# alberto-paparella/MusicRecommendation

Hardware: AMD Instinct MI355X
Metric: scored (test-user,song) pairs/sec, ItemBasedModel, 1/2/4/8 MI355X + mAP@10 (higher is better)
Workload: dtype int64

## Files before the change

include/mr_engine.h:

```cpp
#ifndef MR_ENGINE_H
#define MR_ENGINE_H

#include <stdint.h>
#include <stddef.h>

#ifdef __cplusplus
extern "C" {
#endif

#define MR_OK          0
#define MR_E_INVALID  -1
#define MR_E_HIP      -2
#define MR_E_OOM      -3
#define MR_E_STATE    -4
#define MR_E_IO       -5
#define MR_E_PARSE    -6
#define MR_E_RCCL     -7

#define MR_UBM 0
#define MR_IBM 1

#define MR_OUT_F32 0
#define MR_OUT_F64 1

// ... 17 lines not shown
  int32_t song_lo;
  int32_t song_hi;
  int32_t block_songs;
  int32_t out_dtype;
  int32_t topk;
  int32_t dense;
  int32_t time_kernels;
  int32_t stage1;
  int32_t stage1_chunk;
  int32_t train_order;
  int32_t topk_lists;
  int32_t ibm_route;
  int32_t reserved[2];
} mr_options;

typedef struct mr_ctx mr_ctx;

int mr_options_default(mr_options* opt);

int mr_create(const mr_options* opt, mr_ctx** out);
int mr_destroy(mr_ctx* ctx);

int mr_load(mr_ctx* ctx, const mr_dataset* d);

int mr_shard_info(const mr_ctx* ctx, int32_t* song_lo, int32_t* song_hi, int32_t* n_test_users);

int mr_launch_info(const mr_ctx* ctx, int32_t* shape, int32_t* block_songs, int32_t* n_tiles);

int mr_batch_info(const mr_ctx* ctx, int32_t* batch, int32_t* chunk, int32_t* n_chunks);

int mr_route_info(const mr_ctx* ctx, int32_t* route, int32_t* n_rows, int64_t* pool_entries);

int mr_topk_mode(const mr_ctx* ctx, int32_t* candidate_only);

int mr_cooc_stats(mr_ctx* ctx, int64_t* index_nnz, int64_t* consumed, int64_t* build_reads);

typedef struct mr_cooc_bytes_t {
  int64_t heavy_rows, light_rows;
  int64_t heavy_reads, light_reads;
  int64_t heavy_index_bytes, light_index_bytes;
  int64_t heavy_visits;
  int64_t consumed_bytes;
  int64_t group_tiles;
  int64_t n_groups;
  int64_t index_sparse_entries, index_dense_songs;
  int64_t consumed_sparse_entries, consumed_dense_songs;
} mr_cooc_bytes_t;
int mr_cooc_bytes(mr_ctx* ctx, mr_cooc_bytes_t* out);

int mr_shard_tile_songs(const mr_options* opt, int32_t n_train_users, int32_t n_test_users,
                        int32_t* tile_songs);

int mr_shard_tile_songs_n(const mr_options* opt, int32_t n_train_users, int32_t n_test_users, int32_t n_songs,
                          int32_t n_shards, int32_t* tile_songs);

int mr_run(mr_ctx* ctx, int model);
int mr_sync(mr_ctx* ctx);

int mr_graph_capture(mr_ctx* ctx, int model, int32_t n_steps);
int mr_graph_launch(mr_ctx* ctx);

int mr_device_outputs(const mr_ctx* ctx, void** dense, int32_t** topk_songs,
                      int64_t** topk_keys, double** topk_scores);

int mr_run_into(mr_ctx* ctx, int model, void* dense_dev);

// ... 125 lines not shown
```

musicrecommendation_amd/_lib.py:

```python
from __future__ import annotations

import ctypes
import os
from ctypes import POINTER, c_char_p, c_double, c_int, c_int32, c_int64, c_void_p

_HERE = os.path.dirname(os.path.abspath(__file__))
_VARIANT = os.environ.get("MR_ENGINE_LIB", "")
LIB_PATH = os.path.join(_HERE, f"libmr_engine_{_VARIANT}.so" if _VARIANT else "libmr_engine.so")

MR_OK = 0
MR_E_INVALID = -1
MR_E_HIP = -2
MR_E_OOM = -3
MR_E_STATE = -4
MR_E_IO = -5
MR_E_PARSE = -6
MR_E_RCCL = -7
MR_TRANSPORT_AUTO, MR_TRANSPORT_COPY, MR_TRANSPORT_RCCL = 0, 1, 2
MR_UBM = 0
MR_IBM = 1
STAGE1 = {"auto": 0, "fused": 1, "separate": 2, "wide": 4}
SHAPES = {0: "separate", 1: "fused", 3: "wide"}
MR_OUT_F32 = 0
MR_OUT_F64 = 1
# ... 67 lines not shown
        ("te_songs", c_void_p),
        ("stream", c_void_p),
    ]


class MrCoocBytes(ctypes.Structure):
    _fields_ = [(n, c_int64) for n in ("heavy_rows", "light_rows", "heavy_reads", "light_reads",
                                       "heavy_index_bytes", "light_index_bytes", "heavy_visits", "consumed_bytes",
                                       "group_tiles", "n_groups", "index_sparse_entries", "index_dense_songs",
                                       "consumed_sparse_entries", "consumed_dense_songs")]


MR_COMB_LINEAR = 0
MR_COMB_AGGREGATION = 1
MR_COMB_STOCHASTIC = 2


class EngineError(RuntimeError):
    def __init__(self, code: int, where: str, msg: str):
        super().__init__(f"{where}: {_ERRNAMES.get(code, code)}: {msg}")
        self.code = code


SIGNATURES = {
    "mr_options_default": (c_int, [POINTER(MrOptions)]),
    "mr_create": (c_int, [POINTER(MrOptions), POINTER(c_void_p)]),
    "mr_destroy": (c_int, [c_void_p]),
    "mr_load": (c_int, [c_void_p, POINTER(MrDataset)]),
    "mr_shard_info": (c_int, [c_void_p, POINTER(c_int32), POINTER(c_int32), POINTER(c_int32)]),
    "mr_launch_info": (c_int, [c_void_p, POINTER(c_int32), POINTER(c_int32), POINTER(c_int32)]),
    "mr_batch_info": (c_int, [c_void_p, POINTER(c_int32), POINTER(c_int32), POINTER(c_int32)]),
    "mr_route_info": (c_int, [c_void_p, POINTER(c_int32), POINTER(c_int32), POINTER(c_int64)]),
    "mr_topk_mode": (c_int, [c_void_p, POINTER(c_int32)]),
    "mr_cooc_stats": (c_int, [c_void_p, POINTER(c_int64), POINTER(c_int64), POINTER(c_int64)]),
    "mr_cooc_bytes": (c_int, [c_void_p, POINTER(MrCoocBytes)]),
    "mr_shard_tile_songs": (c_int, [POINTER(MrOptions), c_int32, c_int32, POINTER(c_int32)]),
    "mr_shard_tile_songs_n": (c_int, [POINTER(MrOptions), c_int32, c_int32, c_int32, c_int32, POINTER(c_int32)]),
    "mr_run": (c_int, [c_void_p, c_int]),
    "mr_sync": (c_int, [c_void_p]),
    "mr_graph_capture": (c_int, [c_void_p, c_int, c_int32]),
    "mr_graph_launch": (c_int, [c_void_p]),
    "mr_device_outputs": (c_int, [c_void_p, POINTER(c_void_p), POINTER(c_void_p), POINTER(c_void_p), POINTER(c_void_p)]),
    "mr_score_dense": (c_int, [c_void_p, c_int, c_void_p]),
    "mr_topk": (c_int, [c_void_p, c_int, c_int, c_void_p, c_void_p, c_void_p]),
    "mr_copy_dense": (c_int, [c_void_p, c_void_p]),
    "mr_copy_topk": (c_int, [c_void_p, c_void_p, c_void_p, c_void_p]),
    "mr_copy_topk_device": (c_int, [c_void_p, c_void_p, c_void_p]),
    "mr_copy_topk_device_async": (c_int, [c_void_p, c_void_p, c_void_p]),
    "mr_topk_merge_device_async": (c_int, [c_void_p, c_int32, c_int32, c_int32, c_void_p, c_void_p, c_void_p, c_void_p,
                                           c_void_p]),
    "mr_topk_record_bytes": (c_int, [c_int32, c_int32, POINTER(c_int64)]),
    "mr_topk_merge_records_async": (c_int, [c_void_p, c_int32, c_int32, c_int32, c_void_p, c_int64, c_void_p, c_void_p,
                                            c_void_p]),
    "mr_topk_merge_host": (c_int, [c_int32, c_int32, c_int32, c_void_p, c_void_p, c_void_p, c_void_p, c_void_p, c_void_p]),
    "mr_topk_merge_device": (c_int, [c_void_p, c_int32, c_int32, c_int32, c_void_p, c_void_p, c_void_p, c_void_p, c_void_p, c_void_p]),
    "mr_kernel_times": (c_int, [c_void_p, c_int32, POINTER(c_int64), POINTER(c_double), c_int32]),
    "mr_debug_stamps": (c_int, [c_void_p, c_void_p, c_int64]),
    "mr_timing_begin": (c_int, [c_void_p]),
    "mr_timing_stop": (c_int, [c_void_p]),
    "mr_timing_end": (c_int, [c_void_p, POINTER(c_int64), POINTER(c_double)]),
    "mr_stream": (c_void_p, [c_void_p]),
    "mr_run_into": (c_int, [c_void_p, c_int, c_void_p]),
    "mr_view_get": (c_int, [c_void_p, POINTER(MrView)]),
    "mr_topk_dense_device": (c_int, [c_void_p, c_void_p, c_int32]),
    "mr_combine_device": (c_int, [c_void_p, c_int, c_double, ctypes.c_uint64, c_int64, c_int64, c_void_p, c_void_p, c_void_p]),
    "mr_combine_all_device": (c_int, [c_void_p, c_double, c_double, c_double, ctypes.c_uint64, c_int64, c_int64,
# ... 78 lines not shown
```

musicrecommendation_amd/csrc/mr_engine.hip:

```cpp
#include <hip/hip_runtime.h>

#include <algorithm>
#include <atomic>
#include <climits>
#include <cmath>
#include <cstdarg>
#include <cstdio>
#include <cstdlib>
#include <cstring>
#include <limits>
#include <mutex>
#include <string>
#include <vector>

#ifndef MR_TILE_ROWS
#define MR_TILE_ROWS 32
#endif

#include "mr_engine.h"
#include "mr_internal.h"
#include "mr_par.h"


namespace {
// ... 893 lines not shown
  const uint2* te_sched;
  const long long* sched_off;
  const double* sqrt_c;
  const long long* trs_off;
  const int* trs_users;
  const long long* q_song;
  const double* sqrt_tr;
  const double* sqrt_te;
  int cap;
  int chunk, n_chunks;
  int n_users, xcd_remap;
  int merge_rows;
  const int* nbr_v;
  const long long* nbr_q;
  const int* nbr_cnt;
  void* dense_out;
  long long* cand_key;
  int* cand_song;
  unsigned* counter;
  long long* top_key;
  int* top_song;
  double* top_score;
  long long* stamps;
  int topk_lists;
  int n_rows, nseg;
  const int* te_row;
  const long long* seg_off;
  const int* seg_len;
  const unsigned* pool;
  unsigned long long* mm_key;
  int mm_n;
  int cand;
  const float* rsq_c;
};

template <int MODEL, typename OutT, bool FUSED>
__global__ __launch_bounds__(kThreads) void k_score(ScoreParams p) {
  extern __shared__ __align__(16) unsigned char smem_raw[];
  const int bs = p.block_songs;
  const ScoreLds L = score_lds(bs, FUSED ? p.n_tr : 0, p.topk, p.n_tiles, FUSED ? 0 : p.n_chunks);
  unsigned long long* acc = reinterpret_cast<unsigned long long*>(smem_raw + L.acc);
  unsigned* heard = reinterpret_cast<unsigned*>(smem_raw + L.heard);
  long long* wk = reinterpret_cast<long long*>(smem_raw + L.wk);
  int* ws = reinterpret_cast<int*>(smem_raw + L.ws);
  long long* fk = reinterpret_cast<long long*>(smem_raw + L.fk);
  int* fs = reinterpret_cast<int*>(smem_raw + L.fs);
  int* flag = reinterpret_cast<int*>(smem_raw + L.flag);

  int tile = blockIdx.x;
  int bu = blockIdx.y;
  if (p.xcd_remap) {
    const int lin = blockIdx.y * gridDim.x + blockIdx.x;
    const int slot = lin >> 3;
    bu = (slot / p.n_tiles) * 8 + (lin & 7);
    tile = slot % p.n_tiles;
    if (bu >= p.n_users) return;
  }
  const int u = p.user0 + bu;
  const int tid = threadIdx.x;
  const int blo = p.song_lo + tile * bs;
  const int bhi = min(p.song_hi, blo + bs);
  const int bw = bhi - blo;
  const double two_f = ldexp(1.0, p.frac_bits);
#ifdef MR_STAMPS
  long long* sb = p.stamps ? p.stamps + ((size_t)blockIdx.y * gridDim.x + blockIdx.x) * kStampSlots : nullptr;
#endif
// ... 668 lines not shown
      ba = a > ba ? a : ba;
      ap[e] = a;
    }
  }
  const long long mk = be >= 0 ? (long long)__float_as_uint(ba) : kKeyNone;
  const int ms = be >= 0 ? blo + tid + be * NT : INT_MAX;
  MR_STAMP(3);
  long long tk;
  int tsg;
  block_tau<NT, NG>(k, mk, ms, gm, tk, tsg, sb);
  int* counter = reinterpret_cast<int*>(reinterpret_cast<long long*>(gm) + NG + 1) + NG + 1;
  int* crank = counter + 1 + NG;
  const float thr = __uint_as_float((unsigned)tk) * (1.f - 0x1p-17f);
  const double inv_f = ldexp(1.0, -p.frac_bits);
  unsigned sm = 0u;
#pragma unroll
  for (int e = 0; e < EMAX; ++e) sm |= ap[e] >= thr ? 1u << e : 0u;
  while (sm) {
    const int e = __builtin_ctz(sm);
    sm &= sm - 1u;
    const int i = tid + e * NT;
    double score = (double)(long long)acc[i] * inv_f;
    if (MODEL == MR_IBM) score = score / p.sqrt_c[blo + i];
    const int pos = atomicAdd(counter, 1);
    if (pos < cap) { ck[pos] = __double_as_longlong(score); cs[pos] = blo + i; }
  }
  __syncthreads();
  stamp_at(sb, 11);
  const int nc = *counter;
  if (nc > cap) return false;
  rank_survivors<NT>(nc, k, ck, cs, crank, fk, fs);
  return true;
}
constexpr int kCandE = 20;

template <int MODEL, typename OutT, int NT, int KS, bool COOC>
__global__ __launch_bounds__(NT) void k_score_wide(ScoreParams p) {
  constexpr int NW = NT / 64;
  extern __shared__ __align__(16) unsigned char smem_raw[];
  const int bs = p.block_songs;
  const WideLds<NT> L = wide_lds<NT>(bs, p.topk, p.n_chunks);
  unsigned long long* acc = reinterpret_cast<unsigned long long*>(smem_raw + L.acc);
  unsigned* heard = reinterpret_cast<unsigned*>(smem_raw + L.heard);
  int* cpre = reinterpret_cast<int*>(smem_raw + L.cpre);
  int* s_scan = reinterpret_cast<int*>(smem_raw + L.s_scan);

  const int lin = blockIdx.y * gridDim.x + blockIdx.x;
  const int slot = lin >> 3;
  int bu, tile;
  if (p.xcd_remap == 2) {
    const int per_xcd = (gridDim.x * gridDim.y) >> 3;
    const int pidx = (lin & 7) * per_xcd + slot;
    tile = pidx / gridDim.y;
    bu = pidx - tile * gridDim.y;
  } else if (p.xcd_remap == 3) {
    tile = lin / gridDim.y;
    bu = lin - tile * gridDim.y;
  } else {
    bu = (slot / p.n_tiles) * 8 + (lin & 7);
    tile = slot % p.n_tiles;
  }
  if (bu >= p.n_users) return;
  const int u = p.user0 + bu;
  const int tid = threadIdx.x, lane = tid & 63, w = tid >> 6;
  const int blo = p.song_lo + tile * bs;
  const int bhi = min(p.song_hi, blo + bs);
  const int bw = bhi - blo;
  MR_STAMP(0);

  constexpr bool kPF = COOC && MR_COOC_PF > 0;
  constexpr int PF = kPF ? MR_COOC_PF : 1;
  double scp[PF];
  if constexpr (kPF) {
#pragma unroll
    for (int e = 0; e < PF; ++e) {
      const int i = tid + e * NT;
      scp[e] = i < bw ? p.sqrt_c[blo + i] : 1.0;
    }
  }
  constexpr bool kDPF = COOC && MR_COOC_DPF;
  int pf_r = -1, pf_s = 0, pf_sl = 0;
  long long pf_off = 0;
  unsigned long long pf_q = 0ull;
  if constexpr (kDPF) {
    const long long a = p.te_off[u];
    if (tid < min<long long>(p.nseg, p.te_off[u + 1] - a)) {
      pf_r = p.te_row[a + tid];
      pf_s = p.te_songs[a + tid];
    }
  }
  auto zero_acc = [&]() {
#if MR_WIDE_Z16
    for (int i = tid; 2 * i < bw; i += NT) reinterpret_cast<ulonglong2*>(acc)[i] = make_ulonglong2(0ull, 0ull);
#else
    for (int i = tid; i < bw; i += NT) acc[i] = 0ull;
#endif
  };
  if (!(COOC && MR_COOC_NOZERO) || p.te_off[u + 1] == p.te_off[u]) zero_acc();
  if constexpr (kDPF) {
    if (pf_r >= 0) {
      pf_sl = p.seg_len[(size_t)tile * p.n_rows + pf_r];
      pf_off = p.seg_off[(size_t)tile * p.n_rows + pf_r];
      pf_q = (unsigned long long)p.q_song[pf_s];
    }
  }
  for (int i = tid; i < bs / 32; i += NT) heard[i] = 0u;
  __syncthreads();
  for (long long i = p.te_off[u] + tid; i < p.te_off[u + 1]; i += NT) {
    const int s = p.te_songs[i];
    if (s >= blo && s < bhi) atomicOr(&heard[(s - blo) >> 5], 1u << ((s - blo) & 31));
  }
  const int nch = p.n_chunks;
  int cnt = 0;
  if constexpr (!COOC) {
    for (int c0 = 0; c0 < nch; c0 += NT) {
      const int cc = c0 + tid;
      const int x = cc < nch ? p.nbr_cnt[(size_t)bu * nch + cc] : 0;
      int tot;
      const int pre = block_excl_scan_nt<NT>(x, &tot, s_scan);
      if (cc < nch) cpre[cc] = cnt + pre;
      cnt += tot;
    }
    if (tid == 0) cpre[nch] = cnt;
  }
  __syncthreads();
  MR_STAMP(1);

  bool have_rv = false;
  float pre_rv[MR_CAND_EB];
  if constexpr (COOC) {
    long long* m_off = reinterpret_cast<long long*>(smem_raw + L.wk);
    unsigned long long* m_q = reinterpret_cast<unsigned long long*>(m_off + p.nseg);
    long long* d_off = reinterpret_cast<long long*>(m_q + p.nseg);
    unsigned long long* d_q = reinterpret_cast<unsigned long long*>(d_off + p.nseg);
    int* m_pre = reinterpret_cast<int*>(d_q + p.nseg);
    int* d_fmt = m_pre + p.nseg + 1;
    const long long t0 = p.te_off[u], t1 = p.te_off[u + 1];
    const int* slen = p.seg_len + (size_t)tile * p.n_rows;
    const long long* soff = p.seg_off + (size_t)tile * p.n_rows;
    for (long long c0 = t0; c0 < t1; c0 += p.nseg) {
      const int ns = (int)min<long long>(p.nseg, t1 - c0);
      int len = 0, isd = 0, fmt = 0;
      long long off = 0, tail_off = -1;
      unsigned long long q = 0ull;
      if (tid < ns) {
        int r, sl = 0;
        if (kDPF && c0 == t0) {
          r = pf_r;
          sl = pf_sl;
          off = pf_off;
          q = pf_q;
        } else {
          r = p.te_row[c0 + tid];
          if (r >= 0) {
            sl = slen[r];
            off = soff[r];
            q = (unsigned long long)p.q_song[p.te_songs[c0 + tid]];
          }
        }
// ... 201 lines not shown
    int cur = 0;
    auto load_list = [&](int k0, int (&v)[R], unsigned long long (&q)[R]) {
#pragma unroll
      for (int r = 0; r < R; ++r) {
        const int k = k0 + r * NT;
        v[r] = -1;
        q[r] = 0ull;
        if (k < cnt) {
          while (cur + 1 < nch && cpre[cur + 1] <= k) ++cur;
          const size_t idx = (size_t)cur * p.chunk + (k - cpre[cur]);
          v[r] = nv[idx];
          q[r] = (unsigned long long)nq[idx];
        }
      }
    };
    walk_tile_lists<NT, R, kSeg, unsigned long long>(tid, cnt, load_list, p.toff + (size_t)tile * p.n_tr, p.tsongs,
                                                     [&](unsigned x, unsigned long long q) { atomicAdd(&acc[x], q); });
  }
  __syncthreads();
  MR_STAMP(2);

  long long* wk = reinterpret_cast<long long*>(smem_raw + L.wk);
  int* ws = reinterpret_cast<int*>(smem_raw + L.ws);
  long long* fk = reinterpret_cast<long long*>(smem_raw + L.fk);
  int* fs = reinterpret_cast<int*>(smem_raw + L.fs);
  const int k = KS == 10 ? 10 : p.topk;
  bool have = false;
#ifdef MR_STAMPS
  long long* sbp = p.stamps ? p.stamps + ((size_t)blockIdx.y * gridDim.x + blockIdx.x) * kStampSlots : nullptr;
#else
  long long* sbp = nullptr;
#endif
  if (p.cand) {
    have = wide_cand_topk<MODEL, NT, kCandE>(p, acc, heard, blo, bw, k, smem_raw + L.gm, wk, ws,
                                             min(256, NW * k), fk, fs, sbp, have_rv, pre_rv);
    MR_STAMP(6);
  }
  if (!have) {
  const double inv_f = ldexp(1.0, -p.frac_bits);
  OutT* out = reinterpret_cast<OutT*>(p.dense_out) + (size_t)u * p.width + (blo - p.song_lo);
  long long mk = kKeyNone;
  int ms = INT_MAX;
  OutT lmn = (OutT)INFINITY, lmx = (OutT)-INFINITY;
  auto store = [&](int i, bool h, double score) {
    const OutT o = h ? (OutT)NAN : (OutT)score;
    out[i] = o;
    if (!h) {
      lmn = o < lmn ? o : lmn;
      lmx = o > lmx ? o : lmx;
    }
  };
  constexpr int EB = MR_WIDE_EB;
  int i_start = tid;
  if constexpr (kPF) {
#pragma unroll
    for (int e = 0; e < PF; ++e) {
      const int i = tid + e * NT;
      if (i >= bw) continue;
      const bool h = (heard[i >> 5] >> (i & 31)) & 1u;
      double score = (double)(long long)acc[i] * inv_f;
      score = score / scp[e];
      if (p.dense) store(i, h, score);
      const long long key = h ? kKeyNone : __double_as_longlong(score);
      acc[i] = (unsigned long long)key;
      if (key >= 0) take_if_before(mk, ms, key, blo + i);
    }
    i_start = tid + PF * NT;
  }
// ... 1157 lines not shown

}

struct mr_ctx {
  mr_options opt{};
  int dev_share = 1;
  hipStream_t stream = nullptr;
  bool loaded = false;
  bool ran = false;
  bool fused = false;
  int shape = kShapeSeparate;
  int last_model = -1;
  int n_tr = 0, n_te = 0, n_s = 0;
  int song_lo = 0, song_hi = 0, width = 0;
  int block_songs = 0, n_tiles = 0;
  int cap = 0, batch = 0;
  int chunk = 1, n_chunks = 1;
  size_t score_lds = 0, nbr_lds = 0, merge_lds = 0, wide_lds = 0;
  ScoreKernel score_kernel[2] = {nullptr, nullptr};
  NbrKernel nbr_kernel[2] = {nullptr, nullptr};
  DevBuf<long long> tr_off, te_off, trs_off, q_song, cand_key, top_key, nbr_q;
  DevBuf<int> te_songs, trs_users, toff, nbr_v, nbr_cnt, cand_song, top_song;
  DevBuf<unsigned short> tsongs;
  DevBuf<unsigned> tpack;
  DevBuf<int2> te_rng;
  DevBuf<long long> te_q;
  DevBuf<uint2> te_sched;
  DevBuf<long long> sched_off;
  DevBuf<int> sbound;
  DevBuf<unsigned> counter;
  DevBuf<double> sqrt_c, sqrt_tr, sqrt_te, top_score;
  DevBuf<float> rsq_c;
  bool cand_on = false;
  DevBuf<unsigned char> dense;
  DevBuf<long long> stamps;
  hipEvent_t stage_ev[2] = {nullptr, nullptr};
  static constexpr int kRing = 1024;
  std::vector<hipEvent_t> ring;
  int ring_used = 0;
  bool ring_has_stage1[kRing] = {};
  long long launches[3] = {0, 0, 0};
  double ms[3] = {0, 0, 0};
  hipEvent_t win[2] = {nullptr, nullptr};
  bool win_open = false;
  bool win_stopped = false;
  void* dense_override = nullptr;
  DevBuf<unsigned long long> mm_key;
  bool mm_on = false, mm_valid = false;
  hipGraph_t graph = nullptr;
  hipGraphExec_t graph_exec = nullptr;
  int graph_steps = 0;
  DevBuf<unsigned> flag;
  long long win_launches = 0;
  int ibm_route = 1;
  int cooc_nt = 1024;
  size_t cooc_score_lds = 0;
  int n_rows = 0, nseg = 0;
  long long pool_cap = 0;
  size_t cooc_lds = 0;
  ScoreKernel cooc_kernel = nullptr;
  DevBuf<int> row_song, te_row, seg_len;
  DevBuf<long long> row_base, seg_off;
  DevBuf<unsigned> pool;
  DevBuf<unsigned> row_nnz;
  std::vector<int32_t> row_users;
  std::vector<int64_t> row_reads;
  std::vector<int32_t> row_listeners;
  std::vector<uint8_t> row_light;
  long long build_reads = 0;
  bool cooc_ran = false;
  hipStream_t side[2] = {nullptr, nullptr};
  hipEvent_t side_fork = nullptr, side_join[2] = {nullptr, nullptr};
  int n_heavy = 0, n_light = 0;
  int n_light_tier[6] = {0, 0, 0, 0, 0, 0};
  int n_heavy32 = 0;
  int n_big16 = 0, tcap16 = 0, tcap32 = 0;
  int dense_div = 0, force32 = 0;
  unsigned sat = 255;
  size_t bstamp_off = 0;
  size_t lstamp_off = 0;
  DevBuf<int> rows_order, row_slots;
  DevBuf<int4> rdesc;
  DevBuf<long long> sr_off;
  DevBuf<unsigned> sr_songs;
  DevBuf<unsigned> urec;
  DevBuf<unsigned> lrec;
  DevBuf<uint2> llrec;
  int grp = 0, n_grp = 0, urec_words = 0, lrec_words = 0;
  int group_nt = 1024;

  void release_data() {
    tr_off.release(); te_off.release(); trs_off.release(); q_song.release();
    cand_key.release(); top_key.release(); nbr_q.release();
    tsongs.release(); tpack.release(); te_rng.release(); te_q.release(); te_sched.release(); sched_off.release(); te_songs.release(); trs_users.release(); toff.release(); sbound.release();
    nbr_v.release(); nbr_cnt.release(); cand_song.release(); top_song.release();
    counter.release();
    sqrt_c.release(); sqrt_tr.release(); sqrt_te.release(); top_score.release();
    rsq_c.release(); cand_on = false;
    dense.release();
    mm_key.release(); mm_on = mm_valid = false;
    stamps.release();
    flag.release();
    row_song.release(); te_row.release(); seg_len.release(); row_base.release(); seg_off.release();
    pool.release();
    rows_order.release(); row_slots.release(); sr_off.release(); sr_songs.release(); row_nnz.release();
    urec.release(); lrec.release(); llrec.release(); rdesc.release(); grp = n_grp = urec_words = lrec_words = 0;
    row_users.clear(); row_reads.clear(); row_listeners.clear(); row_light.clear();
    build_reads = 0; cooc_ran = false;
    ibm_route = 1; n_rows = 0; nseg = 0; pool_cap = 0; cooc_kernel = nullptr; n_heavy = n_light = n_heavy32 = 0;
    for (int& x : n_light_tier) x = 0;
    if (graph_exec) (void)hipGraphExecDestroy(graph_exec);
    if (graph) (void)hipGraphDestroy(graph);
    graph_exec = nullptr;
    graph = nullptr;
    graph_steps = 0;
    loaded = ran = false;
  }
};

namespace {

template <class F>
int64_t first_bad(int64_t n, F&& bad, int64_t grain = 1 << 14) {
  std::atomic<int64_t> best{INT64_MAX};
  mr_par::parallel_for(n, [&](int64_t lo, int64_t hi, int) {
    for (int64_t i = lo; i < hi && i < best.load(std::memory_order_relaxed); ++i)
      if (bad(i)) {
        int64_t cur = best.load();
        while (i < cur && !best.compare_exchange_weak(cur, i)) {}
        return;
      }
// ... 824 lines not shown
        c->urec.release();
      }
      MR_HIP(hipStreamSynchronize(st));
    }
  }
  if (k > 0) {
    const int cand_users = !wide ? n_te : route == 2 ? std::max(batch, std::min(n_te, 65528)) : batch;
    const size_t nc = (size_t)cand_users * n_tiles * k;
    if ((rc = dev_alloc(c->cand_key, nc))) return rc;
    if ((rc = dev_alloc(c->cand_song, nc))) return rc;
    const size_t nk = (size_t)n_te * k;
    if ((rc = dev_alloc(c->top_key, (size_t)topk_record_bytes(nk) / 8))) return rc;
    c->top_song.p = reinterpret_cast<int*>(c->top_key.p + nk);
    c->top_song.n = nk;
    c->top_song.own = false;
    if ((rc = dev_alloc(c->top_score, (size_t)n_te * k))) return rc;
    const size_t n_ctr = wide ? (size_t)n_te : (size_t)n_te * kCounterStride;
    if ((rc = dev_alloc(c->counter, n_ctr))) return rc;
    MR_HIP(hipMemsetAsync(c->counter.p, 0, n_ctr * sizeof(unsigned), st));
  }
  const size_t esz = c->opt.out_dtype == MR_OUT_F64 ? 8 : 4;
  if ((rc = dev_alloc(c->dense, c->opt.dense ? (size_t)n_te * width * esz : 1))) return rc;
  if ((rc = dev_alloc(c->flag, 1))) return rc;

  c->fused = fused;
  c->shape = shape;
  c->ibm_route = route;
  c->cooc_nt = cooc_nt_opt();
  {
    const char* e = std::getenv("MR_WIDE_CAND");
    const int nt = route == 2 ? c->cooc_nt : kWideThreads;
    c->cand_on = wide && !c->opt.dense && k >= 1 && k <= nt / 16 && !c->opt.topk_lists && bs <= kCandE * nt &&
                 !(e && e[0] == '0');
  }
  c->wide_lds = wide ? (size_t)wide_lds<kWideThreads>(bs, k, n_chunks).total : 0;
  pick_kernels<MR_UBM>(c);
  pick_kernels<MR_IBM>(c);
  c->score_lds = wide ? c->wide_lds
                      : (size_t)score_lds(bs, fused ? n_tr : 0, k, n_tiles, fused ? 0 : n_chunks).total;
  if (c->score_lds > 160 * 1024)
    return fail(MR_E_INVALID, "scoring kernel needs %zu B of LDS (> 160 KiB): lower block_songs or topk",
                c->score_lds);
  c->nbr_lds = (size_t)align16(chunk * 8) + kThreads * 16 + (kThreads + 4 + kWaves) * 4;
  for (int m = 0; m < 2; ++m) {
    MR_HIP(hipFuncSetAttribute((const void*)c->score_kernel[m], hipFuncAttributeMaxDynamicSharedMemorySize,
                               (int)c->score_lds));
    MR_HIP(hipFuncSetAttribute((const void*)c->nbr_kernel[m], hipFuncAttributeMaxDynamicSharedMemorySize,
                               (int)c->nbr_lds));
  }
  if (route == 2) {
    c->n_rows = (int)row_song.size();
    c->pool_cap = pool_cap;
    const WideLds<kWideThreads> WL = c->cooc_nt == 512 ? wide_lds<512>(bs, k, n_chunks).as_wide()
                                                       : wide_lds<kWideThreads>(bs, k, n_chunks);
    c->cooc_score_lds = (size_t)WL.total;
    c->nseg = std::min(std::min(c->cooc_nt, (WL.total - WL.wk - 8) / 40), 255);
    if (c->nseg < 16) return fail(MR_E_INVALID, "co-listening route: no LDS for row descriptors");
    c->cooc_lds = (size_t)cooc_build_lds<false>(bs);
    c->n_heavy = (int)heavy_rows.size();
    c->build_reads = 0;
    for (int64_t x : row_reads) c->build_reads += x;
    c->row_users.assign(row_song.size(), 0);
    for (size_t i = 0; i < (size_t)d->te_off[n_te]; ++i)
      if (te_row[i] >= 0) c->row_users[te_row[i]]++;
    c->row_reads = row_reads;
    c->row_listeners.resize(row_song.size());
// ... 40 lines not shown
  MR_HIP(hipMemsetAsync(c->stamps.p, 0, n_stamps * 8, st));
  c->bstamp_off = (size_t)n_tiles * stamp_users * kStampSlots;
  c->lstamp_off = c->bstamp_off + build_wgs * 8;
#endif
  MR_HIP(hipStreamSynchronize(st));
  trace("upload");

  c->n_tr = n_tr; c->n_te = n_te; c->n_s = n_s;
  c->song_lo = lo; c->song_hi = hi; c->width = width;
  c->block_songs = bs; c->n_tiles = n_tiles;
  c->cap = cap; c->batch = batch;
  c->chunk = chunk; c->n_chunks = n_chunks;
  c->loaded = true;
  c->ran = false;
  return MR_OK;
}

int mr_route_info(const mr_ctx* c, int32_t* route, int32_t* n_rows, int64_t* pool_entries) {
  if (!c) return fail(MR_E_INVALID, "null context");
  if (!c->loaded) return fail(MR_E_STATE, "mr_route_info before mr_load");
  if (route) *route = c->ibm_route;
  if (n_rows) *n_rows = c->n_rows;
  if (pool_entries) *pool_entries = c->pool_cap;
  return MR_OK;
}

int mr_topk_mode(const mr_ctx* c, int32_t* candidate_only) {
  if (!c || !candidate_only) return fail(MR_E_INVALID, "null argument");
  if (!c->loaded) return fail(MR_E_STATE, "mr_topk_mode before mr_load");
  *candidate_only = c->cand_on ? 1 : 0;
  return MR_OK;
}

int mr_cooc_stats(mr_ctx* c, int64_t* index_nnz, int64_t* consumed, int64_t* build_reads) {
  if (!c) return fail(MR_E_INVALID, "null context");
  if (!c->loaded || c->ibm_route != 2) return fail(MR_E_STATE, "mr_cooc_stats needs a context on ibm_route 2");
  if (!c->cooc_ran) return fail(MR_E_STATE, "mr_cooc_stats before an ibm run");
  MR_HIP(hipSetDevice(c->opt.device));
  std::vector<unsigned> nnz((size_t)std::max(1, c->n_rows), 0u);
  if (c->n_rows > 0)
    MR_HIP(hipMemcpyAsync(nnz.data(), c->row_nnz.p, (size_t)c->n_rows * 4, hipMemcpyDeviceToHost, c->stream));
  MR_HIP(hipStreamSynchronize(c->stream));
  int64_t tot = 0, use = 0;
  for (int r = 0; r < c->n_rows; ++r) {
    tot += nnz[r];
    use += (int64_t)nnz[r] * c->row_users[r];
  }
  if (index_nnz) *index_nnz = tot;
  if (consumed) *consumed = use;
  if (build_reads) *build_reads = c->build_reads;
  return MR_OK;
}

int mr_cooc_bytes(mr_ctx* c, mr_cooc_bytes_t* out) {
  if (!c || !out) return fail(MR_E_INVALID, "null argument");
  if (!c->loaded || c->ibm_route != 2) return fail(MR_E_STATE, "mr_cooc_bytes needs a context on ibm_route 2");
  if (!c->cooc_ran) return fail(MR_E_STATE, "mr_cooc_bytes before an ibm run");
  MR_HIP(hipSetDevice(c->opt.device));
  const int nr = c->n_rows, nt = c->n_tiles;
  std::vector<int32_t> len((size_t)std::max(1, nr) * nt, 0);
  if (nr > 0)
    MR_HIP(hipMemcpyAsync(len.data(), c->seg_len.p, (size_t)nr * nt * 4, hipMemcpyDeviceToHost, c->stream));
  MR_HIP(hipStreamSynchronize(c->stream));
  mr_cooc_bytes_t b{};
  for (int r = 0; r < nr; ++r) {
    int64_t seg = 0;
// ... 176 lines not shown
      if (int rc2 = light_tier_call(t, ls, c->n_light_tier[t], &lp, lp)) return rc2;
      lr += c->n_light_tier[t];
    }
    if (side)
      for (int i = 0; i < 2; ++i) {
        MR_HIP(hipEventRecord(c->side_join[i], c->side[i]));
        MR_HIP(hipStreamWaitEvent(st, c->side_join[i], 0));
      }
  }
  if (timed) MR_HIP(hipEventRecord(ev[1], st));
  for (int y0 = 0; y0 < c->n_te; y0 += 65528) {
    const int ny = std::min(65528, c->n_te - y0);
    const int remap = wide_map_opt();
    ScoreParams sp{};
    sp.chunk = c->chunk; sp.n_chunks = c->n_chunks;
    sp.n_users = ny; sp.xcd_remap = remap;
    sp.merge_rows = merge_rows_opt();
    sp.n_tr = c->n_tr;
    sp.user0 = y0;
    sp.song_lo = c->song_lo; sp.song_hi = c->song_hi; sp.width = c->width;
    sp.block_songs = c->block_songs; sp.n_tiles = c->n_tiles;
    sp.frac_bits = c->opt.frac_bits; sp.topk = k; sp.dense = c->opt.dense;
    sp.te_off = c->te_off.p; sp.te_songs = c->te_songs.p;
    sp.sqrt_c = c->sqrt_c.p; sp.q_song = c->q_song.p;
    sp.n_rows = c->n_rows; sp.nseg = c->nseg;
    sp.te_row = c->te_row.p; sp.seg_off = c->seg_off.p; sp.seg_len = c->seg_len.p; sp.pool = c->pool.p;
    sp.dense_out = c->dense_override ? c->dense_override : (void*)c->dense.p;
    sp.cand_key = c->cand_key.p; sp.cand_song = c->cand_song.p; sp.counter = c->counter.p;
    sp.top_key = c->top_key.p; sp.top_song = c->top_song.p; sp.top_score = c->top_score.p;
    sp.stamps = y0 == 0 ? c->stamps.p : nullptr;
    sp.topk_lists = c->opt.topk_lists;
    if (c->mm_on) { sp.mm_key = c->mm_key.p; sp.mm_n = c->n_te; }
    sp.cand = c->cand_on && !sp.mm_key; sp.rsq_c = c->rsq_c.p;
    hipLaunchKernelGGL(c->cooc_kernel, dim3(c->n_tiles, (ny + 7) / 8 * 8), dim3(c->cooc_nt), c->cooc_score_lds, st, sp);
    MR_HIP(hipGetLastError());
    if (k > 0 && c->n_tiles > 1) {
      MergeParams mp{c->n_tiles, k, k, (long long)c->n_tiles * k, (long long)k, (long long)k, c->cand_key.p,
                     c->cand_song.p, c->top_key.p + (size_t)y0 * k, c->top_song.p + (size_t)y0 * k,
                     c->top_score.p + (size_t)y0 * k};
      hipLaunchKernelGGL(k_topk_merge, dim3(ny), dim3(kThreads), c->merge_lds, st, mp);
      MR_HIP(hipGetLastError());
    }
    if (c->win_open) c->win_launches++;
  }
  if (timed) MR_HIP(hipEventRecord(ev[2], st));
  return MR_OK;
}

int ensure_nbr(mr_ctx* c) {
  if (c->shape == kShapeFused || (c->nbr_v.p && c->nbr_q.p && c->nbr_cnt.p)) return MR_OK;
  int rc;
  if ((rc = dev_alloc(c->nbr_v, (size_t)c->batch * c->cap))) return rc;
  if ((rc = dev_alloc(c->nbr_q, (size_t)c->batch * c->cap))) return rc;
  if ((rc = dev_alloc(c->nbr_cnt, (size_t)c->batch * c->n_chunks))) return rc;
  return MR_OK;
}

int run_model(mr_ctx* c, int model) {
  if (model == MR_IBM && c->ibm_route == 2) {
    c->cooc_ran = true;
    return run_cooc(c);
  }
  hipStream_t st = c->stream;
  const bool timed = c->opt.time_kernels != 0;
  const int k = c->opt.topk;
  for (int user0 = 0; user0 < c->n_te; user0 += c->batch) {
    const int nb = std::min(c->batch, c->n_te - user0);
    hipEvent_t* ev = nullptr;
    if (timed) {
      if (c->ring_used == mr_ctx::kRing) {
        int rc = flush_timing(c);
        if (rc) return rc;
// ... 27 lines not shown
      const bool wide = c->shape == kShapeWide;
      int remap = (c->shape == kShapeSeparate && c->n_tiles > 1) || wide;
      if (wide) remap = wide_map_opt();
      const int gy = remap ? (ny + 7) / 8 * 8 : ny;
      ScoreParams sp{};
      sp.chunk = c->chunk; sp.n_chunks = c->n_chunks;
      sp.n_users = ny; sp.xcd_remap = remap;
      sp.merge_rows = merge_rows_opt();
      sp.n_tr = c->n_tr;
      sp.user0 = user0 + y0;
      sp.song_lo = c->song_lo; sp.song_hi = c->song_hi; sp.width = c->width;
      sp.block_songs = c->block_songs; sp.n_tiles = c->n_tiles;
      sp.frac_bits = c->opt.frac_bits; sp.topk = k; sp.dense = c->opt.dense;
      sp.te_off = c->te_off.p; sp.te_songs = c->te_songs.p;
      sp.toff = c->toff.p; sp.tsongs = c->tsongs.p; sp.tpack = c->tpack.p; sp.sqrt_c = c->sqrt_c.p;
      sp.te_rng = c->te_rng.p; sp.te_q = c->te_q.p;
      sp.te_sched = c->te_sched.p; sp.sched_off = c->sched_off.p;
#ifdef MR_NO_TERNG
      sp.te_rng = nullptr;
#endif
      sp.trs_off = c->trs_off.p; sp.trs_users = c->trs_users.p; sp.q_song = c->q_song.p;
      sp.sqrt_tr = c->sqrt_tr.p; sp.sqrt_te = c->sqrt_te.p;
      sp.cap = c->cap;
      sp.nbr_v = c->fused ? nullptr : c->nbr_v.p + (size_t)y0 * c->cap;
      sp.nbr_q = c->fused ? nullptr : c->nbr_q.p + (size_t)y0 * c->cap;
      sp.nbr_cnt = c->fused ? nullptr : c->nbr_cnt.p + (size_t)y0 * c->n_chunks;
      sp.dense_out = c->dense_override ? c->dense_override : (void*)c->dense.p;
      sp.cand_key = c->cand_key.p; sp.cand_song = c->cand_song.p; sp.counter = c->counter.p;
      sp.top_key = c->top_key.p; sp.top_song = c->top_song.p; sp.top_score = c->top_score.p;
      sp.stamps = c->stamps.p ? c->stamps.p + (size_t)y0 * c->n_tiles * kStampSlots : nullptr;
      sp.topk_lists = c->opt.topk_lists;
      if (c->mm_on && wide) { sp.mm_key = c->mm_key.p; sp.mm_n = c->n_te; }
      sp.cand = wide && c->cand_on && !sp.mm_key; sp.rsq_c = c->rsq_c.p;
      hipLaunchKernelGGL(c->score_kernel[model], dim3(c->n_tiles, gy), dim3(wide ? kWideThreads : kThreads),
                         c->score_lds, st, sp);
      MR_HIP(hipGetLastError());
      if (wide && k > 0 && c->n_tiles > 1) {
        MergeParams mp{c->n_tiles, k, k, (long long)c->n_tiles * k, (long long)k, (long long)k, c->cand_key.p, c->cand_song.p,
                       c->top_key.p + (size_t)(user0 + y0) * k, c->top_song.p + (size_t)(user0 + y0) * k,
                       c->top_score.p + (size_t)(user0 + y0) * k};
        hipLaunchKernelGGL(k_topk_merge, dim3(ny), dim3(kThreads), c->merge_lds, st, mp);
        MR_HIP(hipGetLastError());
      }
      if (c->win_open) c->win_launches++;
    }
    if (timed) MR_HIP(hipEventRecord(ev[2], st));
  }
  return MR_OK;
}

}

namespace mr_internal {

namespace {
struct StagePool {
  std::mutex m;
  void* buf[2] = {nullptr, nullptr};
};
StagePool& stage_pool() {
  static StagePool* p = new StagePool;
  return *p;
}
}

int d2h_staged(mr_ctx* c, void* dst, size_t dpitch, const void* src, size_t spitch, size_t row_bytes, size_t rows) {
  const size_t total = row_bytes * rows;
  if (total == 0) return MR_OK;
  hipPointerAttribute_t attr;
  const bool pinned = hipPointerGetAttributes(&attr, dst) == hipSuccess && attr.type == hipMemoryTypeHost;
  (void)hipGetLastError();
  constexpr size_t kStage = (size_t)64 << 20;
  if (pinned || total < ((size_t)8 << 20) || row_bytes > kStage) {
// ... 404 lines not shown
```

musicrecommendation_amd/engine.py:

```python
from __future__ import annotations

import ctypes
from typing import Optional, Tuple, Union

import numpy as np

from . import _lib
from .dataset import Dataset

MODELS = {"ubm": _lib.MR_UBM, "ibm": _lib.MR_IBM, _lib.MR_UBM: _lib.MR_UBM, _lib.MR_IBM: _lib.MR_IBM}
KERNELS = {"neighbours": 0, "score": 1}
IBM_ROUTES = {"auto": 0, "two_hop": 1, "cooc": 2}


def model_id(model: Union[str, int]) -> int:
    try:
        return MODELS[model]
    except KeyError:
        raise ValueError(f"unknown model {model!r}: use 'ubm' or 'ibm'") from None


class Engine:
    def __init__(self, dataset: Dataset, *, device: int = 0, frac_bits: int = 32, song_lo: int = 0,
                 song_hi: int = 0, block_songs: int = 0, out_dtype: str = "f32", topk: int = 10,
# ... 21 lines not shown
        self.dtype = np.float32 if out_dtype == "f32" else np.float64
        self._h = ctypes.c_void_p()
        _lib.check(self._L.mr_create(ctypes.byref(opt), ctypes.byref(self._h)), "mr_create")
        self.dataset = dataset
        try:
            cd = dataset.c_struct()
            _lib.check(self._L.mr_load(self._h, ctypes.byref(cd)), "mr_load")
        except Exception:
            self.close()
            raise
        lo, hi, nte = ctypes.c_int32(), ctypes.c_int32(), ctypes.c_int32()
        _lib.check(self._L.mr_shard_info(self._h, ctypes.byref(lo), ctypes.byref(hi), ctypes.byref(nte)),
                   "mr_shard_info")
        self.song_lo, self.song_hi, self.n_test = lo.value, hi.value, nte.value
        self.width = self.song_hi - self.song_lo
        self.topk_k = topk
        fz, bsz, nt = ctypes.c_int32(), ctypes.c_int32(), ctypes.c_int32()
        _lib.check(self._L.mr_launch_info(self._h, ctypes.byref(fz), ctypes.byref(bsz), ctypes.byref(nt)),
                   "mr_launch_info")
        self.shape = _lib.SHAPES[fz.value]
        self.fused, self.block_songs, self.n_tiles = self.shape == "fused", bsz.value, nt.value
        b, ch, nch = ctypes.c_int32(), ctypes.c_int32(), ctypes.c_int32()
        _lib.check(self._L.mr_batch_info(self._h, ctypes.byref(b), ctypes.byref(ch), ctypes.byref(nch)),
                   "mr_batch_info")
        self.batch, self.stage1_chunk, self.n_chunks = b.value, ch.value, nch.value
        rt, nr, pe = ctypes.c_int32(), ctypes.c_int32(), ctypes.c_int64()
        _lib.check(self._L.mr_route_info(self._h, ctypes.byref(rt), ctypes.byref(nr), ctypes.byref(pe)),
                   "mr_route_info")
        self.ibm_route = {1: "two_hop", 2: "cooc"}[rt.value]
        self.cooc_rows, self.cooc_pool_entries = nr.value, pe.value
        co = ctypes.c_int32()
        _lib.check(self._L.mr_topk_mode(self._h, ctypes.byref(co)), "mr_topk_mode")
        self.candidate_topk = bool(co.value)

    def close(self) -> None:
        if getattr(self, "_h", None) is not None and self._h.value:
            self._L.mr_destroy(self._h)
            self._h = ctypes.c_void_p()

    def __enter__(self):
        return self

    def __exit__(self, *exc):
        self.close()

    def __del__(self):
        try:
            self.close()
        except Exception:
            pass

    def run(self, model: Union[str, int]) -> None:
        _lib.check(self._L.mr_run(self._h, model_id(model)), "mr_run")

    def cooc_stats(self) -> Tuple[int, int, int]:
        a, b, c = ctypes.c_int64(), ctypes.c_int64(), ctypes.c_int64()
        _lib.check(self._L.mr_cooc_stats(self._h, ctypes.byref(a), ctypes.byref(b), ctypes.byref(c)), "mr_cooc_stats")
        return a.value, b.value, c.value

    def cooc_bytes(self) -> dict:
        b = _lib.MrCoocBytes()
        _lib.check(self._L.mr_cooc_bytes(self._h, ctypes.byref(b)), "mr_cooc_bytes")
        return {name: int(getattr(b, name)) for name, _t in _lib.MrCoocBytes._fields_}

    def sync(self) -> None:
        _lib.check(self._L.mr_sync(self._h), "mr_sync")
# ... 191 lines not shown
```

Measured before the change: 16.98 billion.

## Score first tile slab, merge, then threshold remaining tiles against provisional top-k

The wide candidate top-k path now runs in two launches. The first covers a small slab of song tiles, its per-tile lists are merged into a provisional top-k, and the second launch scores the remaining tiles using the current k-th key as a pruning threshold. The threshold lets most tiles skip the full candidate ranking through a cheap float filter, with a wave-level rank when few survivors remain. In exchange it adds an extra kernel launch and merge, serialises the first slab before the rest, and falls back to the old path if the survivor buffer overflows.

```diff
diff --git a/include/mr_engine.h b/include/mr_engine.h
--- a/include/mr_engine.h
+++ b/include/mr_engine.h
@@ -73,6 +73,8 @@
 int mr_route_info(const mr_ctx* ctx, int32_t* route, int32_t* n_rows, int64_t* pool_entries);
 
 int mr_topk_mode(const mr_ctx* ctx, int32_t* candidate_only);
+
+int mr_wide_slab(const mr_ctx* ctx, int32_t* slab_tiles);
 
 int mr_cooc_stats(mr_ctx* ctx, int64_t* index_nnz, int64_t* consumed, int64_t* build_reads);
 
diff --git a/musicrecommendation_amd/_lib.py b/musicrecommendation_amd/_lib.py
--- a/musicrecommendation_amd/_lib.py
+++ b/musicrecommendation_amd/_lib.py
@@ -123,6 +123,7 @@
     "mr_batch_info": (c_int, [c_void_p, POINTER(c_int32), POINTER(c_int32), POINTER(c_int32)]),
     "mr_route_info": (c_int, [c_void_p, POINTER(c_int32), POINTER(c_int32), POINTER(c_int64)]),
     "mr_topk_mode": (c_int, [c_void_p, POINTER(c_int32)]),
+    "mr_wide_slab": (c_int, [c_void_p, POINTER(c_int32)]),
     "mr_cooc_stats": (c_int, [c_void_p, POINTER(c_int64), POINTER(c_int64), POINTER(c_int64)]),
     "mr_cooc_bytes": (c_int, [c_void_p, POINTER(MrCoocBytes)]),
     "mr_shard_tile_songs": (c_int, [POINTER(MrOptions), c_int32, c_int32, POINTER(c_int32)]),
diff --git a/musicrecommendation_amd/csrc/mr_engine.hip b/musicrecommendation_amd/csrc/mr_engine.hip
--- a/musicrecommendation_amd/csrc/mr_engine.hip
+++ b/musicrecommendation_amd/csrc/mr_engine.hip
@@ -949,6 +949,8 @@
   int mm_n;
   int cand;
   const float* rsq_c;
+  int tile0, slab_tiles;
+  const long long* thr_key;
 };
 
 template <int MODEL, typename OutT, bool FUSED>
@@ -1683,7 +1685,95 @@
   rank_survivors<NT>(nc, k, ck, cs, crank, fk, fs);
   return true;
 }
+
+#ifndef MR_SLAB_EB
+#define MR_SLAB_EB 4
+#endif
+#ifndef MR_SLAB_WAVE_RANK
+#define MR_SLAB_WAVE_RANK 16
+#endif
+template <int MODEL, int NT, int EMAX>
+__device__ __forceinline__ bool wide_slab_topk(const ScoreParams& p, const unsigned long long* acc,
+                                               const unsigned* heard, int blo, int bw, int k, unsigned char* gm,
+                                               int* counter, long long* ck, int* cs, int cap, const TopkDst& dst,
+                                               long long* fk, int* fs, long long* sb, bool have_rv,
+                                               const float (&pre_rv)[MR_CAND_EB], float thr) {
+  constexpr int NG = NT / 16;
+  const int tid = threadIdx.x;
+  int* crank = reinterpret_cast<int*>(reinterpret_cast<long long*>(gm) + NG + 1) + NG + 1 + 1 + NG;
+  if (tid < 256) crank[tid] = 0;
+  const double inv_f = ldexp(1.0, -p.frac_bits);
+  unsigned sm = 0u;
+  unsigned hw[EMAX];
+#pragma unroll
+  for (int e = 0; e < EMAX; ++e) {
+    const int i = tid + e * NT;
+    hw[e] = i < bw ? heard[i >> 5] : ~0u;
+  }
+  constexpr int EB = MR_SLAB_EB;
+#pragma unroll
+  for (int e0 = 0; e0 < EMAX; e0 += EB) {
+    unsigned long long av[EB];
+    float rv[EB];
+#pragma unroll
+    for (int j = 0; j < EB; ++j) {
+      const int i = tid + (e0 + j) * NT;
+      av[j] = 0ull;
+      rv[j] = 0.f;
+      if (e0 + j < EMAX && i < bw) {
+        av[j] = acc[i];
+        rv[j] = MODEL != MR_IBM ? 1.f : (e0 + j < MR_CAND_EB && have_rv) ? pre_rv[e0 + j] : p.rsq_c[blo + i];
+      }
+    }
+#pragma unroll
+    for (int j = 0; j < EB; ++j) {
+      const int e = e0 + j;
+      if (e >= EMAX) continue;
+      float a = -1.f;
+      if (!((hw[e] >> (tid & 31)) & 1u)) {
+        const float hi = (float)(unsigned)(av[j] >> 32), lo = (float)(unsigned)av[j];
+        a = __fmaf_rn(hi, 4294967296.f, lo) * rv[j];
+      }
+      sm |= a >= thr ? 1u << e : 0u;
+    }
+  }
+  while (sm) {
+    const int e = __builtin_ctz(sm);
+    sm &= sm - 1u;
+    const int i = tid + e * NT;
+    double score = (double)(long long)acc[i] * inv_f;
+    if (MODEL == MR_IBM) score = score / p.sqrt_c[blo + i];
+    const int pos = atomicAdd(counter, 1);
+    if (pos < cap) { ck[pos] = __double_as_longlong(score); cs[pos] = blo + i; }
+  }
+  MR_STAMP(3);
+  __syncthreads();
+  stamp_at(sb, 9);
+  stamp_at(sb, 10);
+  stamp_at(sb, 11);
+  const int nc = *counter;
+  stamp_val(sb, 15, nc + 1);
+  if (nc > cap) return false;
+  if (nc <= MR_SLAB_WAVE_RANK) {
+    if (tid < 64) {
+      const long long mine = tid < nc ? ck[tid] : kKeyNone;
+      const int mines = tid < nc ? cs[tid] : INT_MAX;
+      int r = 0;
+      for (int j = 0; j < nc; ++j) r += cand_before(ck[j], cs[j], mine, mines) ? 1 : 0;
+      if (tid < nc) {
+        if (r < k) topk_dst_write(dst, r, mine, mines);
+      } else if (tid < k) {
+        topk_dst_write(dst, tid, kKeyNone, -1);
+      }
+    }
+    return true;
+  }
+  rank_survivors<NT>(nc, k, ck, cs, crank, fk, fs, dst);
+  return true;
+}
 constexpr int kCandE = 20;
+constexpr int kSlabTiles = 4;
+constexpr int kSlabMinTiles = 8;
 
 template <int MODEL, typename OutT, int NT, int KS, bool COOC>
 __global__ __launch_bounds__(NT) void k_score_wide(ScoreParams p) {
@@ -1708,16 +1798,18 @@
     tile = lin / gridDim.y;
     bu = lin - tile * gridDim.y;
   } else {
-    bu = (slot / p.n_tiles) * 8 + (lin & 7);
-    tile = slot % p.n_tiles;
+    bu = (slot / p.slab_tiles) * 8 + (lin & 7);
+    tile = slot % p.slab_tiles;
   }
   if (bu >= p.n_users) return;
+  tile += p.tile0;
   const int u = p.user0 + bu;
   const int tid = threadIdx.x, lane = tid & 63, w = tid >> 6;
   const int blo = p.song_lo + tile * bs;
   const int bhi = min(p.song_hi, blo + bs);
   const int bw = bhi - blo;
   MR_STAMP(0);
+  const long long sk = p.thr_key ? p.thr_key[(size_t)u * p.topk] : kKeyNone;
 
   constexpr bool kPF = COOC && MR_COOC_PF > 0;
   constexpr int PF = kPF ? MR_COOC_PF : 1;
@@ -1776,6 +1868,11 @@
   }
   __syncthreads();
   MR_STAMP(1);
+  int* slab_cnt = COOC ? cpre : s_scan;
+  float thr = -1.f;
+  if (sk >= 0) thr = (float)(__longlong_as_double(sk) * ldexp(1.0, p.frac_bits)) * (1.f - 0x1p-17f);
+  thr = __uint_as_float(__builtin_amdgcn_readfirstlane(__float_as_uint(thr)));
+  if (tid == 0) *slab_cnt = 0;
 
   bool have_rv = false;
   float pre_rv[MR_CAND_EB];
@@ -2043,8 +2140,24 @@
   long long* sbp = nullptr;
 #endif
   if (p.cand) {
-    have = wide_cand_topk<MODEL, NT, kCandE>(p, acc, heard, blo, bw, k, smem_raw + L.gm, wk, ws,
-                                             min(256, NW * k), fk, fs, sbp, have_rv, pre_rv);
+    stamp_val(sbp, 15, 0);
+    if (thr >= 0.f) {
+      TopkDst dst;
+      dst.key = p.cand_key + ((size_t)bu * p.n_tiles + tile) * k;
+      dst.song = p.cand_song + ((size_t)bu * p.n_tiles + tile) * k;
+      if (wide_slab_topk<MODEL, NT, kCandE>(p, acc, heard, blo, bw, k, smem_raw + L.gm, slab_cnt, wk, ws,
+                                            min(256, NW * k), dst, fk, fs, sbp, have_rv, pre_rv, thr)) {
+        MR_STAMP(6);
+        MR_STAMP(7);
+        MR_STAMP(8);
+        MR_STAMP(4);
+        MR_STAMP(5);
+        return;
+      }
+    }
+    if (!have)
+      have = wide_cand_topk<MODEL, NT, kCandE>(p, acc, heard, blo, bw, k, smem_raw + L.gm, wk, ws,
+                                               min(256, NW * k), fk, fs, sbp, have_rv, pre_rv);
     MR_STAMP(6);
   }
   if (!have) {
@@ -3268,6 +3381,7 @@
   DevBuf<double> sqrt_c, sqrt_tr, sqrt_te, top_score;
   DevBuf<float> rsq_c;
   bool cand_on = false;
+  int slab = 0;
   DevBuf<unsigned char> dense;
   DevBuf<long long> stamps;
   hipEvent_t stage_ev[2] = {nullptr, nullptr};
@@ -3332,7 +3446,7 @@
     nbr_v.release(); nbr_cnt.release(); cand_song.release(); top_song.release();
     counter.release();
     sqrt_c.release(); sqrt_tr.release(); sqrt_te.release(); top_score.release();
-    rsq_c.release(); cand_on = false;
+    rsq_c.release(); cand_on = false; slab = 0;
     dense.release();
     mm_key.release(); mm_on = mm_valid = false;
     stamps.release();
@@ -4223,6 +4337,9 @@
     const int nt = route == 2 ? c->cooc_nt : kWideThreads;
     c->cand_on = wide && !c->opt.dense && k >= 1 && k <= nt / 16 && !c->opt.topk_lists && bs <= kCandE * nt &&
                  !(e && e[0] == '0');
+    const char* s = std::getenv("MR_WIDE_SLAB");
+    const int want = s ? std::atoi(s) : n_tiles >= kSlabMinTiles ? kSlabTiles : 0;
+    c->slab = c->cand_on && want >= 1 && want < n_tiles ? want : 0;
   }
   c->wide_lds = wide ? (size_t)wide_lds<kWideThreads>(bs, k, n_chunks).total : 0;
   pick_kernels<MR_UBM>(c);
@@ -4329,6 +4446,13 @@
   return MR_OK;
 }
 
+int mr_wide_slab(const mr_ctx* c, int32_t* slab_tiles) {
+  if (!c || !slab_tiles) return fail(MR_E_INVALID, "null argument");
+  if (!c->loaded) return fail(MR_E_STATE, "mr_wide_slab before mr_load");
+  *slab_tiles = c->slab;
+  return MR_OK;
+}
+
 int mr_cooc_stats(mr_ctx* c, int64_t* index_nnz, int64_t* consumed, int64_t* build_reads) {
   if (!c) return fail(MR_E_INVALID, "null context");
   if (!c->loaded || c->ibm_route != 2) return fail(MR_E_STATE, "mr_cooc_stats needs a context on ibm_route 2");
@@ -4571,12 +4695,26 @@
     sp.topk_lists = c->opt.topk_lists;
     if (c->mm_on) { sp.mm_key = c->mm_key.p; sp.mm_n = c->n_te; }
     sp.cand = c->cand_on && !sp.mm_key; sp.rsq_c = c->rsq_c.p;
-    hipLaunchKernelGGL(c->cooc_kernel, dim3(c->n_tiles, (ny + 7) / 8 * 8), dim3(c->cooc_nt), c->cooc_score_lds, st, sp);
+    const int gy = (ny + 7) / 8 * 8;
+    MergeParams mp{c->n_tiles, k, k, (long long)c->n_tiles * k, (long long)k, (long long)k, c->cand_key.p,
+                   c->cand_song.p, c->top_key.p + (size_t)y0 * k, c->top_song.p + (size_t)y0 * k,
+                   c->top_score.p + (size_t)y0 * k};
+    const int slab = sp.cand ? c->slab : 0;
+    sp.tile0 = 0; sp.slab_tiles = slab ? slab : c->n_tiles;
+    hipLaunchKernelGGL(c->cooc_kernel, dim3(sp.slab_tiles, gy), dim3(c->cooc_nt), c->cooc_score_lds, st, sp);
     MR_HIP(hipGetLastError());
+    if (slab) {
+      MergeParams m1 = mp;
+      m1.n_lists = slab;
+      hipLaunchKernelGGL(k_topk_merge, dim3(ny), dim3(kThreads), c->merge_lds, st, m1);
+      MR_HIP(hipGetLastError());
+      sp.tile0 = slab; sp.slab_tiles = c->n_tiles - slab;
+      sp.thr_key = c->top_key.p + (k - 1);
+      if (sp.stamps) sp.stamps += (size_t)slab * gy * kStampSlots;
+      hipLaunchKernelGGL(c->cooc_kernel, dim3(sp.slab_tiles, gy), dim3(c->cooc_nt), c->cooc_score_lds, st, sp);
+      MR_HIP(hipGetLastError());
+    }
     if (k > 0 && c->n_tiles > 1) {
-      MergeParams mp{c->n_tiles, k, k, (long long)c->n_tiles * k, (long long)k, (long long)k, c->cand_key.p,
-                     c->cand_song.p, c->top_key.p + (size_t)y0 * k, c->top_song.p + (size_t)y0 * k,
-                     c->top_score.p + (size_t)y0 * k};
       hipLaunchKernelGGL(k_topk_merge, dim3(ny), dim3(kThreads), c->merge_lds, st, mp);
       MR_HIP(hipGetLastError());
     }
@@ -4670,13 +4808,26 @@
       sp.topk_lists = c->opt.topk_lists;
       if (c->mm_on && wide) { sp.mm_key = c->mm_key.p; sp.mm_n = c->n_te; }
       sp.cand = wide && c->cand_on && !sp.mm_key; sp.rsq_c = c->rsq_c.p;
-      hipLaunchKernelGGL(c->score_kernel[model], dim3(c->n_tiles, gy), dim3(wide ? kWideThreads : kThreads),
+      MergeParams mp{c->n_tiles, k, k, (long long)c->n_tiles * k, (long long)k, (long long)k, c->cand_key.p, c->cand_song.p,
+                     c->top_key.p + (size_t)(user0 + y0) * k, c->top_song.p + (size_t)(user0 + y0) * k,
+                     c->top_score.p + (size_t)(user0 + y0) * k};
+      const int slab = sp.cand ? c->slab : 0;
+      sp.tile0 = 0; sp.slab_tiles = slab ? slab : c->n_tiles;
+      hipLaunchKernelGGL(c->score_kernel[model], dim3(sp.slab_tiles, gy), dim3(wide ? kWideThreads : kThreads),
                          c->score_lds, st, sp);
       MR_HIP(hipGetLastError());
+      if (slab) {
+        MergeParams m1 = mp;
+        m1.n_lists = slab;
+        hipLaunchKernelGGL(k_topk_merge, dim3(ny), dim3(kThreads), c->merge_lds, st, m1);
+        MR_HIP(hipGetLastError());
+        sp.tile0 = slab; sp.slab_tiles = c->n_tiles - slab;
+        sp.thr_key = c->top_key.p + (k - 1);
+        if (sp.stamps) sp.stamps += (size_t)slab * gy * kStampSlots;
+        hipLaunchKernelGGL(c->score_kernel[model], dim3(sp.slab_tiles, gy), dim3(kWideThreads), c->score_lds, st, sp);
+        MR_HIP(hipGetLastError());
+      }
       if (wide && k > 0 && c->n_tiles > 1) {
-        MergeParams mp{c->n_tiles, k, k, (long long)c->n_tiles * k, (long long)k, (long long)k, c->cand_key.p, c->cand_song.p,
-                       c->top_key.p + (size_t)(user0 + y0) * k, c->top_song.p + (size_t)(user0 + y0) * k,
-                       c->top_score.p + (size_t)(user0 + y0) * k};
         hipLaunchKernelGGL(k_topk_merge, dim3(ny), dim3(kThreads), c->merge_lds, st, mp);
         MR_HIP(hipGetLastError());
       }
diff --git a/musicrecommendation_amd/engine.py b/musicrecommendation_amd/engine.py
--- a/musicrecommendation_amd/engine.py
+++ b/musicrecommendation_amd/engine.py
@@ -77,6 +77,9 @@
         co = ctypes.c_int32()
         _lib.check(self._L.mr_topk_mode(self._h, ctypes.byref(co)), "mr_topk_mode")
         self.candidate_topk = bool(co.value)
+        sl = ctypes.c_int32()
+        _lib.check(self._L.mr_wide_slab(self._h, ctypes.byref(sl)), "mr_wide_slab")
+        self.wide_slab = sl.value
 
     def close(self) -> None:
         if getattr(self, "_h", None) is not None and self._h.value:
```

After: 16.96 billion. Within noise of the previous version (-0.1%).
